# RKlompUU/fhe-regex

Hardware: AMD Instinct MI355X
Metric: TFHE gate-bootstraps/sec; end-to-end match time for /abc/ on 256-char content (higher is better)
Workload: dtype u64

## Files before the change

fhe-regex_amd/csrc/device.h:

```cpp
#pragma once
#include <cstdint>
#include <vector>

#include "common.h"
#include "owned.h"

namespace fr {

constexpr int MAX_OUT = 8;
enum : int32_t { JOB_MULTI = 0, JOB_DIRECT = 1, JOB_SIGN = 2 };
struct DevGate {
    int32_t n_in;
    int32_t offset;
    int32_t in_slot[16];
    int32_t in_w[16];
    int32_t n_out;
    int32_t direct;
    int32_t out_slot[MAX_OUT];
    uint8_t lut[MAX_OUT][16];
};
static_assert(sizeof(DevGate) == 304, "DevGate layout");
int lut_w_norm2(const uint8_t* lut);

struct DeviceTimers {
// ... 37 lines not shown
    void pack_bools(const DevGate* gates, size_t n, uint64_t* out_host);
    void pack_bools_compact(const DevGate* gates, size_t n, uint16_t* out_host );
    const double* pack_ms() const { return pack_ms_; }
    void encrypt_to_slots(const ClientKey& ck, const uint8_t* msgs, size_t count, const RngKey& key, uint64_t first_block,
                          const int* slots);

    Slots expand_to_slots(const RngKey& mask_key, uint64_t first_block, const uint8_t* bodies, size_t count);
    double expand_ms() const { return expand_ms_; }

    int alloc_slot();
    void free_slot(int s);
    void write_slots(const int* slots, size_t n, const uint64_t* host );
    void read_slot(int slot, uint64_t* host );
    void slots_to_device(const int* slots, size_t n, uint64_t* dst);
    void device_to_slots(const int* slots, size_t n, const uint64_t* src);
    void slots_to_device_async(const int* slots, size_t n, uint64_t* dst);
    void* stream() const { return cur().stream.get(); }
    void zero_slot(int slot);
    size_t arena_slots() const { return next_slot_; }
    size_t arena_free_slots() const { return free_slots_.size(); }

    void run_level(const DevGate* gates, size_t n);
    void run_level_resident(const DevGate* d_gates, const DevGate* host, size_t n, size_t n_refs = 0);
    gpu::DevBuf<DevGate> upload_gates(const DevGate* gates, size_t n, size_t n_refs = 0);
    void bind_content(const int* cmap, size_t n);
    void run_linear(const DevGate& g);
    void sync();

    void set_lanes(int n);
    int match_lanes() const { return (int)lanes_.size(); }
    void enter_lane(int i);
    void leave_lane();
    void set_profiling(int level) { profiling_ = level; }
    DeviceTimers& timers() { return timers_; }

    void keyswitch_host(const uint64_t* in, size_t count, uint64_t* out);
    void blind_rotate_host(const uint64_t* ks_in, const uint8_t* luts, size_t count, uint64_t* out);
    void blind_rotate_multi_host(const uint64_t* ks_in, const uint8_t* luts, int n_out, int direct, uint64_t* out);
    void ring_mul_host(const uint64_t* a, const uint64_t* b, size_t count, uint64_t* out);
    void bench_pbs(const std::vector<DevGate>& gates, int iters, double* br_ms, double* total_ms);

    std::string info() const;

  private:
    struct LaneState {
        gpu::Stream stream;
        gpu::DevBuf<uint64_t> ks;
        gpu::DevBuf<int8_t> dig;
        gpu::DevBuf<DevGate> pk_gates;
        gpu::DevBuf<int8_t> pk_dig;
        gpu::DevBuf<uint64_t> pk_g;
        gpu::DevBuf<uint16_t> pk_c16;
        gpu::DevBuf<double> kpre;
        gpu::StagingRing<int> cmap;
        size_t cmap_n = 0;
        gpu::Event done_ev;
        bool pending = false;
    };
    LaneState lane0_;
    std::vector<LaneState> lanes_;
    int lane_ = 0;
    LaneState& cur() { return lane_ ? lanes_[lane_ - 1] : lane0_; }
    const LaneState& cur() const { return lane_ ? lanes_[lane_ - 1] : lane0_; }
    bool lanes_pending_ = false;
    bool lanes_unsynced_ = false;
    gpu::Event main_ev_;
    std::vector<int> deferred_free_;
    hipStream_t cur_stream();
    void join_lanes();
    void sync_all();
    void ensure_arena(size_t slots);
    void ensure_ks(size_t n);
    void ensure_gates(size_t n);
    void validate_gates(const DevGate* gates, size_t n, size_t n_refs = 0) const;
    void launch_level(const DevGate* d_gates, const DevGate* host, size_t n);
    gpu::Event take_event();
    void resolve_timers();
    void ensure_digits(size_t rows);
    struct LimbKey {
        gpu::DevBuf<uint64_t> rows;
        gpu::DevBuf<int8_t> limbs;
        int KD = 0, ncols = 0, nlc = 0;
        explicit operator bool() const { return rows && limbs; }
        void alloc_rows(int kd, int nc) {
            limbs.reset();
            KD = kd, ncols = nc, nlc = ((nc * 8 + 127) / 128) * 128;
            rows.alloc((size_t)kd * nc);
        }
        void reset() { rows.reset(), limbs.reset(); }
    };
    void build_limbs(LimbKey& key);
    void drop_server_key() {
        ksk_.reset(), d_tbsk_.reset(), d_bsk_.reset(), d_fbsk_[0].reset(), d_fbsk_[1].reset();
        lane0_.kpre.reset();
        for (auto& l : lanes_) l.kpre.reset();
    }
    void drop_packing_key() { pksk_.reset(); }
    struct KsShape {
        int MR;
        size_t padded;
        int MC = 1, GZ = 1;
        bool lds = true;
    };
    KsShape ks_shape(size_t n) const {
        const int MR = n >= ks_mr4_min_ ? 4 : 1;
        return {MR, (n + 32 * MR - 1) / (32 * MR) * (32 * MR)};
    }
    template <int KSB, int KSL>
    void launch_ks_digits(const DevGate* d_gates, size_t n, size_t padded, int8_t* dig, uint64_t* out, int out_n,
                          int out_stride, hipEvent_t ev_start);
    void launch_limb_gemm(const int8_t* dig, const LimbKey& key, size_t n, const KsShape& sh, uint64_t* out,
                          int out_stride, hipEvent_t ev_stop);
    void launch_ks(const DevGate* d_gates, size_t n, uint64_t* d_ks, hipEvent_t ev_start = nullptr,
                   hipEvent_t ev_stop = nullptr);
    void launch_br(const DevGate* d_gates, const uint64_t* d_ks, size_t n, hipEvent_t ev_start = nullptr,
                   hipEvent_t ev_stop = nullptr);
    void run_br_jobs(const uint64_t* ks_in, std::vector<DevGate>& gates, uint64_t* out);
    void init_rns();
    void upload_rns_bsk(const std::vector<uint64_t>& bsk);
    void launch_br_rns(const DevGate* d_gates, const uint64_t* d_ks, size_t n, hipEvent_t ev_start, hipEvent_t ev_stop);
    void init_ks();
    void init_fft();
    void upload_fft_bsk(const std::vector<uint64_t>& bsk);
    void launch_br_fft(const DevGate* d_gates, const uint64_t* d_ks, size_t n, hipStream_t stream,
                       hipEvent_t ev_start = nullptr, hipEvent_t ev_stop = nullptr);
    void build_fourier_bsk();
    double key_load_ms_[5] = {0, 0, 0, 0, 0};
    double pk_load_ms_[3] = {0, 0, 0};
    gpu::StagingRing<uint8_t> xstage_;
    double expand_ms_ = 0;
    void stage_slot_list(const int* slots, size_t n);
    gpu::DevBuf<int> d_slot_list_;

    Params p_;
    int dev_;
    int e_ = 8;
    int e_small_ = 8;
    size_t small_batch_ = 256;
    LimbKey ksk_;
    gpu::DevBuf<uint64_t> d_tbsk_;
    LimbKey pksk_;
    double pack_ms_[4] = {0, 0, 0, 0};
    void pack_launch(const DevGate* gates, size_t n, uint64_t* out_words, uint16_t* out_c16);
    int pk_split_ = 0;
    bool ks_mfma_ = true;
    size_t ks_mr4_min_ = 96;
    int ks_mc_ = 0;
    int ks_split_ = 0;
    int ks_xcd_ = 1;
    bool ks_dig16_ = true;
    bool ks_lds_ = true;
    gpu::DevBuf<uint32_t> d_bsk_;
    gpu::DevBuf<uint32_t> d_tw_;
    int fft_e_ = 4;
    size_t fft_small_ = 256;
    size_t fft_pair_ = SIZE_MAX;
    bool fft_dual_ = false;
    size_t fft_kpre_ = 32;
    gpu::DevBuf<double> d_fbsk_[2];
    static int fbsk_index(int E) { return E == 4 ? 0 : 1; }
    bool fbsk_needed(int E) const { return E == 4 || E == fft_e_; }
    gpu::DevBuf<double> d_ftw_;
    gpu::DevBuf<double> d_fqt_;
    gpu::DevBuf<uint16_t> d_fleaf_;
    gpu::DevBuf<uint64_t> d_arena_;
    std::vector<int> free_slots_;
    size_t next_slot_ = 0;
    gpu::StagingRing<DevGate> gates_;
    struct PendingTimer {
        gpu::Event ev[4];
        size_t gates, outs;
        bool lat, pair, ks;
        bool chain;
    };
    bool latency_shape(size_t n) const;
    bool pair_shape(size_t n) const;
    std::vector<PendingTimer> pending_;
    std::vector<gpu::Event> event_pool_;
    int profiling_ = 0;
    bool timer_chain_ = true;
    DeviceTimers timers_;
    gpu::Event ev_[4];
};

}
```

fhe-regex_amd/csrc/fft_br.hip:

```cpp
#include <hip/hip_ext.h>
#include <hip/hip_runtime.h>

#include <cstring>

#include "device_impl.h"
#include "fft.h"
#include "geo.h"

namespace fr {

template <int M, int E>
using FGeo = NttGeo<M, E, 3, fft_layout_variant(ilog2c(M), ilog2c(E))>;
template <int M, int E>
constexpr int FV = fft_layout_variant(ilog2c(M), ilog2c(E));

__device__ __forceinline__ void cfwd(double2& x, double2& y, double2 c) { fft::fwd_bf(x.x, x.y, y.x, y.y, c.x, c.y); }
__device__ __forceinline__ void cinv(double2& u, double2& v, double2 c) { fft::inv_bf(u.x, u.y, v.x, v.y, c.x, c.y); }

template <int M, int E>
constexpr bool fradix4() {
    return E == 4 && FGeo<M, E>::LOG % 2 == 0;
}
template <int M, int E>
struct FTwr {
    static constexpr int COUNT = fradix4<M, E>() ? FGeo<M, E>::NPH * 3 : FGeo<M, E>::LOG * (E / 2);
    double2 v[COUNT];
};
__device__ __forceinline__ double2 fmul_i(double2 c) { return make_double2(-c.y, c.x); }
__device__ __forceinline__ void cinv_r4(double2 (&x)[4], double2 c, double2 ca, double2 cc) {
    fft::inv_r4(x[0].x, x[0].y, x[1].x, x[1].y, x[2].x, x[2].y, x[3].x, x[3].y, c.x, c.y, ca.x, ca.y, cc.x, cc.y);
}
template <class G, int E, int p, bool REV, class F>
__device__ __forceinline__ void for_butterflies(F&& fn) {
#pragma unroll
    for (int i = 0; i < G::s_end(p) - G::s_begin(p); ++i) {
        const int s = REV ? G::s_end(p) - 1 - i : G::s_begin(p) + i;
        const int dm = 1 << (G::LOG - 1 - s - G::lo(p));
#pragma unroll
        for (int m = 0; m < E; ++m) {
            if (m & dm) continue;
            fn(s, m, dm);
        }
    }
}
template <class G, int p>
__device__ __forceinline__ double2 ftw_at(const double2* tw, int b, int s, int m) {
    return (tw + (b >> (G::LOG - s)))[(1 << s) + (G::template moff<p>(m) >> (G::LOG - s))];
}
template <int M, int E, int p>
__device__ __forceinline__ void ftw_r4(const double2* tw, int tl, double2& c, double2& ca) {
    using G = FGeo<M, E>;
    constexpr int s0 = G::s_begin(p), s1 = s0 + 1;
    const int b = G::template base<p>(tl);
    c = ftw_at<G, p>(tw, b, s0, 0);
    ca = ftw_at<G, p>(tw, b, s1, 0);
// ... 399 lines not shown
        if (src < 0) {
            src += N;
            d = -d;
        }
        acc += (uint64_t)d * row[src];
    }
    return acc;
}

template <int M, int E>
__device__ __forceinline__ void fbr_publish(uint64_t* arow, const double (&alo)[E], const double (&ahi)[E], int tl) {
#pragma unroll
    for (int m = 0; m < E; ++m) {
        const int j = FGeo<M, E>::template idx<0>(tl, m);
        arow[j] = fft::torus_of_acc(alo[m]);
        arow[j + M] = fft::torus_of_acc(ahi[m]);
    }
}
template <int N>
__device__ __forceinline__ void fbr_terms(int tid, int n_out, int kind, const uint8_t* lut, uint32_t* wterms, int* wcnt) {
    if (tid < n_out && kind == JOB_MULTI) wcnt[tid] = lut_terms<N>(lut + 16 * tid, wterms + 16 * tid);
}
template <int N, int K, int NT>
__device__ __forceinline__ void fbr_outputs(int tid, const uint64_t* ab, const DevGate& gate, int n_out, int kind,
                                            const uint32_t* wterms, const int* wcnt, uint64_t* arena, int slot_stride) {
    constexpr int big = K * N;
    if (kind != JOB_MULTI) {
        uint64_t* out = arena + (size_t)gate.out_slot[0] * slot_stride;
        const uint64_t post = kind == JOB_SIGN ? (1ULL << (DELTA_LOG - 1)) : 0;
        for (int c = tid; c <= big; c += NT) {
            const ExtractIdx x = extract_index<N, K>(c);
            const uint64_t v = ab[x.pp * N + x.j];
            out[c] = (x.neg ? (uint64_t)0 - v : v) + (c == big ? post : 0);
        }
        return;
    }
    for (int f = 0; f < n_out; ++f) {
        const uint32_t* tf = wterms + 16 * f;
        const int nt = wcnt[f];
        uint64_t* out = arena + (size_t)gate.out_slot[f] * slot_stride;
        for (int c = tid; c <= big; c += NT) {
            const ExtractIdx x = extract_index<N, K>(c);
            const uint64_t v = w_step64<N>(ab + x.pp * N, tf, nt, x.j);
            out[c] = x.neg ? (uint64_t)0 - v : v;
        }
    }
}

template <int N, int K>
constexpr uint32_t kpre_step_bytes() {
    return 16u * (uint32_t)((K + 1) * (K + 1) * (N / 2));
}

template <int N, int K, int E, bool LAT, int B, bool KP>
__device__ __forceinline__ void fbr_rotate(const uint64_t* ks, int ks_stride, int n, const DevGate* gates, int n_gates,
                                           const double2* bsk, const double2* tw_g, const double2* psi_g,
                                           const uint16_t* leaf_g, uint64_t* arena, int slot_stride, const double2* kpre) {
    constexpr int M = N / 2;
    static_assert(!KP || (LAT && B == 1 && K == 1 && E == 4), "key products: the k = 1 latency shape");
    using G = FGeo<M, E>;
    static_assert(fexchanges_conflict_free<M, E>(), "LDS maps must make every exchange conflict-free");
    static_assert(G::base_matches_geo(), "base<p> must be the index map the LDS-map proofs reason about");
    static_assert(G::key_slot_matches_idx(), "the Fourier key's lane layout is the last-phase layout");
    static_assert(!LAT || E == 4, "the latency shape holds a step's GGSW values in registers: E = 4");
    static_assert(B == 1 || (B == 2 && LAT && K == 1 && E == 4), "pair shape: the k = 1 latency geometry");
    constexpr int NB = E >= 4 ? E / 4 : 1;
    constexpr int T = M / E, NT = (K + 1) * T, LAST = G::NPH - 1, XL = G::XL;
    constexpr int LOG2N2 = G::LOG + 2;
    constexpr bool TWR = fbr_twr<K, LAT>();
    constexpr int BS = (K + 1) * G::NP;
    constexpr bool PSIQ = !LAT || B > 1;
    extern __shared__ __attribute__((aligned(16))) double2 fsm[];
    double2* xbuf = fsm;
    double2* ibuf = LAT ? xbuf + B * BS : xbuf;
    double2* tw = xbuf + (LAT ? 2 : 1) * B * BS;
    constexpr int NPSI = KP ? 0 : PSIQ ? N / 2 : 2 * N;
    double2* psi = tw + (B == 1 ? M : 0);
    double2* twc = psi + NPSI;
    constexpr int NTWC = fbr_twc_entries<N, K, E, LAT>();
    uint8_t* lut = (uint8_t*)(twc + NTWC);
    uint16_t* abar = (uint16_t*)(lut + B * 16 * MAX_OUT);
    uint32_t* wterms = B == 1 ? (uint32_t*)(abar + 1026) : (uint32_t*)ibuf;
    int* wcnt = (int*)(wterms + B * 16 * MAX_OUT);
    uint16_t* nxt = B == 1 ? (uint16_t*)(wcnt + MAX_OUT) : abar + B * 1026;

    const int tid = threadIdx.x;
    const int P = __builtin_amdgcn_readfirstlane(tid / T), tl = tid % T;
    int gb[B];
    bool has[B];
    const uint64_t* in[B];
    int n_out[B], kind[B];
#pragma unroll
    for (int b = 0; b < B; ++b) {
        const int gi = B * (int)blockIdx.x + b;
        has[b] = gi < n_gates;
        gb[b] = has[b] ? gi : B * (int)blockIdx.x;
        in[b] = ks + (size_t)gb[b] * ks_stride;
        n_out[b] = gates[gb[b]].n_out;
        kind[b] = gates[gb[b]].direct;
    }
    if constexpr (B == 1)
        for (int i = tid; i < M; i += NT) tw[i] = tw_g[i];
    for (int i = tid; i < NPSI; i += NT) psi[psi_slot(i)] = psi_g[i];
    for (int i = 1 + tid; i < NTWC; i += NT) {
        const int s0 = 31 - __builtin_clz((unsigned)i), b = i - (1 << s0);
        if (s0 & 1) continue;
        const double2 c = tw_g[i], ca = tw_g[(2 << s0) + 2 * b];
        fft::cmul(c.x, c.y, ca.x, ca.y, twc[i].x, twc[i].y);
    }
    uint32_t bbar[B];
#pragma unroll
    for (int b = 0; b < B; ++b) {
        uint8_t* lb = lut + b * 16 * MAX_OUT;
        uint16_t* ab = abar + b * 1026;
        for (int i = tid; i < 16 * n_out[b]; i += NT) lb[i] = gates[gb[b]].lut[i / 16][i % 16];
        for (int i = tid; i < n; i += NT) ab[i] = (uint16_t)mod_switch(in[b][i], LOG2N2);
        if (tid == 0) ab[n] = 0;
        bbar[b] = mod_switch(in[b][n], LOG2N2);
    }
    uint32_t Lb[NB];
#pragma unroll
    for (int bb = 0; bb < NB; ++bb)
        Lb[bb] = (1u + 4u * (__brev((uint32_t)G::template idx<LAST>(tl, 4 * bb)) >> (32 - G::LOG))) & (uint32_t)(M - 1);
    __syncthreads();

    double alo[B][E], ahi[B][E];
#pragma unroll
    for (int b = 0; b < B; ++b) {
        const bool direct = kind[b] == JOB_DIRECT;
#pragma unroll
        for (int m = 0; m < E; ++m) {
            const int j = G::template idx<0>(tl, m);
            uint64_t v[2];
#pragma unroll
            for (int h = 0; h < 2; ++h) {
                const int s = (j + h * M + (int)bbar[b]) & (2 * N - 1);
                const uint64_t tv = test_poly<N>(s & (N - 1), direct, lut + b * 16 * MAX_OUT);
                v[h] = s < N ? tv : (uint64_t)0 - tv;
            }
            alo[b][m] = P == K ? fft::acc_of_torus(v[0]) : 0.0;
            ahi[b][m] = P == K ? fft::acc_of_torus(v[1]) : 0.0;
        }
    }

    double2* row = xbuf + P * G::NP;
    double2* irow = ibuf + P * G::NP;
    const int bl = G::template base<LAST>(tl);
    double2* row_bl = row + G::template at<XL>(bl);
    const double2* orow_bl[K];
#pragma unroll
    for (int q = 0; q < K; ++q) orow_bl[q] = xbuf + other_row<K>(P, q) * G::NP + G::template at<XL>(bl);
    constexpr uint32_t GG = (uint32_t)(K + 1) * (K + 1) * M;
    const __amdgpu_buffer_rsrc_t rs = bsk_rsrc(bsk);
    const uint32_t lane_off = 16u * (uint32_t)tl;
    const int steps = (n + 1) / 2;
    double2 gv[3][K + 1][LAT && !KP ? E : 1];
    double2 kv[K + 1][KP ? E : 1];
    FTwr<M, TWR ? E : 2> twr;
    if constexpr (TWR) ftw_load_phase<M, E, 0, B == 1 ? false : FR_TW_SGPR_PAIR>(twr, B == 1 ? tw : tw_g, tl);
#ifdef FR_BR_TIMING
    uint64_t tseg[6] = {0, 0, 0, 0, 0, 0};
    uint64_t tlast = __builtin_amdgcn_s_memtime();
    const uint64_t tstart = tlast;
#endif
    auto load_ggsw = [&](int gg, int tt) {
        if constexpr (!KP) {
            const uint32_t sb = (uint32_t)__builtin_amdgcn_readfirstlane(tt) * (3u * GG * 16u);
#pragma unroll
            for (int m = 0; m < E; ++m) {
                gv[gg][0][m] =
                    bsk_load(rs, lane_off, sb + 16u * (gg * GG + (uint32_t)(P * (K + 1) + P) * M + (uint32_t)m * T));
#pragma unroll
                for (int q = 0; q < K; ++q)
                    gv[gg][1 + q][m] = bsk_load(
                        rs, lane_off,
                        sb + 16u * (gg * GG + (uint32_t)(other_row<K>(P, q) * (K + 1) + P) * M + (uint32_t)m * T));
            }
        }
    };
    const __amdgpu_buffer_rsrc_t rk =
        bsk_rsrc(KP ? kpre + (size_t)blockIdx.x * ((size_t)((n + 1) / 2) * (kpre_step_bytes<N, K>() / 16)) : bsk);
    auto load_kp = [&](int tt) {
        if constexpr (KP) {
            const uint32_t sb = (uint32_t)__builtin_amdgcn_readfirstlane(tt) * kpre_step_bytes<N, K>();
#pragma unroll
            for (int r = 0; r <= K; ++r)
#pragma unroll
                for (int m = 0; m < E; ++m)
                    kv[r][m] = bsk_load(rk, lane_off, sb + 16u * (uint32_t)(((P * (K + 1) + r) * E + m) * T));
        }
    };
    constexpr int NPF = KP ? 0 : LAT ? (B > 1 ? FR_PAIR_PF : K == 1 ? FR_LAT_PF : FR_LAT_PF2) : 0;
    constexpr bool LATPF = NPF > 0;
    auto idle = [&](int t) {
        uint32_t z = 0;
#pragma unroll
        for (int b = 0; b < B; ++b) z |= abar[b * 1026 + 2 * t] | abar[b * 1026 + 2 * t + 1];
        return z == 0;
    };
    if constexpr (LATPF || KP) {
        for (int t = tid; t <= steps; t += NT) {
            int tt = t;
            while (tt < steps && idle(tt)) ++tt;
            nxt[t] = (uint16_t)tt;
        }
        __syncthreads();
        const int t0 = __builtin_amdgcn_readfirstlane((int)nxt[0]);
        for (int gg = 0; gg < NPF; ++gg) load_ggsw(gg, t0 < steps ? t0 : 0);
        load_kp(t0 < steps ? t0 : 0);
    }
    for (int t = 0; t < steps; ++t) {
        if (idle(t)) continue;
        BR_STAMP(0);
        const uint32_t sbase = (uint32_t)__builtin_amdgcn_readfirstlane(t) * (3u * GG * 16u);
        constexpr int G_TOP = !LAT || KP || B > 1 ? 3 : (NPF < 2 || K == 1) ? NPF : 3;
        constexpr int G_L1 = !LAT || KP ? 3 : B > 1 ? NPF : G_TOP + 1 < 3 ? G_TOP + 1 : 3;
        constexpr int G_L2 = !LAT || KP ? 3 : B > 1 ? (NPF + 1 < 3 ? NPF + 1 : 3) : G_TOP == 3 ? NPF : G_TOP + 2 < 3 ? G_TOP + 2 : 3;
        constexpr int PH_L1 = B > 1 ? FR_PAIR_LOAD : FR_LAT_LOAD1;
        constexpr int PH_L2 = B > 1 ? FR_PAIR_LOAD2 : FR_LAT_LOAD2;
        static_assert(G_L1 >= 3 || PH_L1 < G::NPH, "FR_PAIR_LOAD / FR_LAT_LOAD1 past the last forward phase");
        static_assert(G_L2 >= 3 || PH_L2 < G::NPH, "FR_PAIR_LOAD2 / FR_LAT_LOAD2 past the last forward phase");
        if constexpr (G_TOP < 3) {
            __builtin_amdgcn_sched_barrier(0);
            load_ggsw(G_TOP, t);
            __builtin_amdgcn_sched_barrier(0);
        }
        uint32_t ei[B], ej[B];
#pragma unroll
        for (int b = 0; b < B; ++b) {
            ei[b] = __builtin_amdgcn_readfirstlane((uint32_t)abar[b * 1026 + 2 * t]);
            ej[b] = __builtin_amdgcn_readfirstlane((uint32_t)abar[b * 1026 + 2 * t + 1]);
        }
        double bre[B][2][NB], bim[B][2][NB];
        auto psi_factors = [&]() {
#pragma unroll
            for (int b = 0; b < B; ++b)
#pragma unroll
                for (int h = 0; h < 2; ++h)
#pragma unroll
                    for (int bb = 0; bb < NB; ++bb)
                        key_psi_base<N, PSIQ>(psi, h == 0 ? ei[b] : ej[b], Lb[bb], bre[b][h][bb], bim[b][h][bb]);
        };
        if constexpr (LAT && B == 1 && !KP) psi_factors();
        double2 x[B][E];
#pragma unroll
        for (int b = 0; b < B; ++b)
#pragma unroll
            for (int m = 0; m < E; ++m)
                x[b][m] = make_double2(fft::acc_digit<23>(alo[b][m]), fft::acc_digit<23>(ahi[b][m]));
        BR_STAMP(1);
        fforward_from<M, E, 0, LAT, TWR, B, BS>(x, row, twr, tw, tl, [&](auto ph) {
            if constexpr (LAT) {
                constexpr int p = decltype(ph)::value;
                if constexpr (p == PH_L1 && G_L1 < 3) {
                    __builtin_amdgcn_sched_barrier(0);
                    load_ggsw(G_L1, t);
                    __builtin_amdgcn_sched_barrier(0);
                }
                if constexpr (p == PH_L2 && G_L2 < 3) {
                    __builtin_amdgcn_sched_barrier(0);
                    load_ggsw(G_L2, t);
                    __builtin_amdgcn_sched_barrier(0);
                }
            }
// ... 5 lines not shown
            for (int m = 0; m < E; ++m) row_bl[b * BS + G::template at<XL>(G::template moff<LAST>(m))] = x[b][m];
        constexpr bool AHEAD = !LAT && E == 8;
        constexpr bool PRE0 = !LAT;
        double2 Bc[3][K + 1];
        if constexpr (PRE0) load_slot<M, T, K>(Bc, rs, sbase, P, 0, lane_off);
        __syncthreads();
        if constexpr (!LAT || B > 1) psi_factors();
#pragma unroll
        for (int m = 0; m < E; ++m) {
            double2 Bn[3][K + 1];
            if constexpr (AHEAD) {
                if (m + 1 < E) load_slot<M, T, K>(Bn, rs, sbase, P, m + 1, lane_off);
                __builtin_amdgcn_sched_barrier(0);
            } else if constexpr (!LAT) {
                if (!PRE0 || m > 0) load_slot<M, T, K>(Bc, rs, sbase, P, m, lane_off);
            }
#pragma unroll
            for (int b = 0; b < B; ++b) {
                const double2 own = x[b][m];
                double2 oth[K];
#pragma unroll
                for (int q = 0; q < K; ++q) oth[q] = orow_bl[q][b * BS + G::template at<XL>(G::template moff<LAST>(m))];
                double kor, koi, kxr[K], kxi[K];
                if constexpr (KP) {
                    kor = kv[0][m].x, koi = kv[0][m].y;
#pragma unroll
                    for (int q = 0; q < K; ++q) kxr[q] = kv[1 + q][m].x, kxi[q] = kv[1 + q][m].y;
                } else {
                    const uint32_t sm = ((m & 1) << 1) | ((m >> 1) & 1);
                    auto key_at = [&](int gg, int r) __attribute__((always_inline)) {
                        return LAT ? gv[gg][r][LAT ? m : 0] : Bc[gg][r];
                    };
                    key_products<K>(bre[b], bim[b], m >> 2, ei[b], ej[b], sm, key_at, kor, koi, kxr, kxi);
                }
                double zr, zi;
                fft::cmul(own.x, own.y, kor, koi, zr, zi);
#pragma unroll
                for (int q = 0; q < K; ++q) fft::cmac(oth[q].x, oth[q].y, kxr[q], kxi[q], zr, zi);
                x[b][m] = make_double2(zr, zi);
            }
            if constexpr (!LAT) {
                __builtin_amdgcn_sched_barrier(0);
            }
            if constexpr (AHEAD) {
#pragma unroll
                for (int gg = 0; gg < 3; ++gg)
#pragma unroll
                    for (int r = 0; r <= K; ++r) Bc[gg][r] = Bn[gg][r];
            }
        }
        if constexpr (LATPF || KP) {
            const int tn = __builtin_amdgcn_readfirstlane((int)nxt[t + 1]);
            __builtin_amdgcn_sched_barrier(0);
            for (int gg = 0; gg < NPF; ++gg) load_ggsw(gg, tn < steps ? tn : t);
            load_kp(tn < steps ? tn : t);
            __builtin_amdgcn_sched_barrier(0);
        }
        BR_STAMP(3);
        finverse_from<M, E, LAST, LAT, TWR, B, BS>(x, irow, twr, tw, twc, tl);
        BR_STAMP(4);
#pragma unroll
        for (int b = 0; b < B; ++b)
#pragma unroll
            for (int m = 0; m < E; ++m) {
                alo[b][m] = fft::acc_reduce<23>(alo[b][m] + x[b][m].x);
                ahi[b][m] = fft::acc_reduce<23>(ahi[b][m] + x[b][m].y);
            }
        BR_STAMP(5);
    }
#ifdef FR_BR_TIMING
    if (blockIdx.x == 0 && tid == 0)
        printf("FBR_TIMING E=%d LAT=%d steps=%d total=%lu digits=%lu fwd=%lu mac=%lu inv=%lu acc=%lu top=%lu\n", E, (int)LAT,
               steps, (unsigned long)(__builtin_amdgcn_s_memtime() - tstart), (unsigned long)tseg[1],
               (unsigned long)tseg[2], (unsigned long)tseg[3], (unsigned long)tseg[4], (unsigned long)tseg[5],
               (unsigned long)tseg[0]);
#endif

    __syncthreads();
    uint64_t* accs = (uint64_t*)xbuf;
    static_assert(B == 1 || 8 * B * (K + 1) * N <= 16 * B * BS, "pair shape: u64 rows inside the forward rows");
#pragma unroll
    for (int b = 0; b < B; ++b) {
        fbr_publish<M, E>(accs + (b * (K + 1) + P) * N, alo[b], ahi[b], tl);
        fbr_terms<N>(tid, n_out[b], kind[b], lut + b * 16 * MAX_OUT, wterms + b * 16 * MAX_OUT, wcnt + b * MAX_OUT);
    }
    __syncthreads();
#pragma unroll
    for (int b = 0; b < B; ++b)
        if (has[b])
            fbr_outputs<N, K, NT>(tid, accs + b * (K + 1) * N, gates[gb[b]], n_out[b], kind[b], wterms + b * 16 * MAX_OUT,
                                  wcnt + b * MAX_OUT, arena, slot_stride);
}

template <int N, int K, int E, bool LAT, int B = 1>
__global__ void __launch_bounds__((fbr_threads<N, K, E>()), (fbr_min_waves<N, K, E, LAT>()))
k_blind_rotate_fft(const uint64_t* __restrict__ ks, int ks_stride, int n, const DevGate* __restrict__ gates,
                   int n_gates, const double2* __restrict__ bsk, const double2* __restrict__ tw_g,
                   const double2* __restrict__ psi_g, const uint16_t* __restrict__ leaf_g, uint64_t* __restrict__ arena,
                   int slot_stride) {
    fbr_rotate<N, K, E, LAT, B, false>(ks, ks_stride, n, gates, n_gates, bsk, tw_g, psi_g, leaf_g, arena, slot_stride,
                                       nullptr);
}
template <int N, int K, int E, bool LAT, int B = 1>
__global__ void __launch_bounds__((fbr_threads<N, K, E>()), (fbr_min_waves<N, K, E, LAT>()))
k_blind_rotate_fft_kp(const uint64_t* __restrict__ ks, int ks_stride, int n, const DevGate* __restrict__ gates,
                      int n_gates, const double2* __restrict__ tw_g, uint64_t* __restrict__ arena, int slot_stride,
                      const double2* __restrict__ kpre) {
    fbr_rotate<N, K, E, LAT, B, true>(ks, ks_stride, n, gates, n_gates, nullptr, tw_g, nullptr, nullptr, arena,
                                      slot_stride, kpre);
}

template <int N>
__global__ void __launch_bounds__(N / 8)
k_key_products(const uint64_t* __restrict__ ks, int ks_stride, int n, int n_gates, const double2* __restrict__ bsk,
               const double2* __restrict__ psi_g, double2* __restrict__ kpre) {
    constexpr int K = 1, E = 4, M = N / 2, T = M / E;
    using G = FGeo<M, E>;
    static_assert(G::key_slot_matches_idx(), "the Fourier key's lane layout is the last-phase layout");
    constexpr int LAST = G::NPH - 1, LOG2N2 = G::LOG + 2;
    constexpr uint32_t GG = (uint32_t)(K + 1) * (K + 1) * M;
    __shared__ __attribute__((aligned(16))) double2 psi[N / 2];
    const int tl = threadIdx.x, t = (int)blockIdx.x, P = (int)blockIdx.y;
    const int steps = (n + 1) / 2;
    for (int i = tl; i < N / 2; i += T) psi[psi_slot(i)] = psi_g[i];
    const __amdgpu_buffer_rsrc_t rs = bsk_rsrc(bsk);
    const uint32_t lane_off = 16u * (uint32_t)tl, sb = (uint32_t)t * (3u * GG * 16u);
    double2 gv[3][K + 1][E];
#pragma unroll
    for (int gg = 0; gg < 3; ++gg)
#pragma unroll
        for (int m = 0; m < E; ++m) {
            gv[gg][0][m] = bsk_load(rs, lane_off, sb + 16u * (gg * GG + (uint32_t)(P * (K + 1) + P) * M + (uint32_t)m * T));
            gv[gg][1][m] = bsk_load(
                rs, lane_off, sb + 16u * (gg * GG + (uint32_t)(other_row<K>(P, 0) * (K + 1) + P) * M + (uint32_t)m * T));
        }
    const uint32_t Lb = (1u + 4u * (__brev((uint32_t)G::template idx<LAST>(tl, 0)) >> (32 - G::LOG))) & (uint32_t)(M - 1);
    __syncthreads();
    for (int b = 0; b < n_gates; ++b) {
        const uint64_t* in = ks + (size_t)b * ks_stride;
        const uint32_t ei = (uint16_t)mod_switch(in[2 * t], LOG2N2);
        const uint32_t ej = 2 * t + 1 < n ? (uint16_t)mod_switch(in[2 * t + 1], LOG2N2) : 0u;
        if ((ei | ej) == 0) continue;
        double br[2][1], bi[2][1];
        key_psi_base<N, true>(psi, ei, Lb, br[0][0], bi[0][0]);
        key_psi_base<N, true>(psi, ej, Lb, br[1][0], bi[1][0]);
        double2* out = kpre + (((size_t)b * steps + t) * (K + 1) + P) * ((K + 1) * M) + tl;
#pragma unroll
        for (int m = 0; m < E; ++m) {
            const uint32_t sm = ((m & 1) << 1) | ((m >> 1) & 1);
            double kor, koi, kxr[K], kxi[K];
            key_products<K>(br, bi, 0, ei, ej, sm, [&](int gg, int r) __attribute__((always_inline)) { return gv[gg][r][m]; },
                            kor, koi, kxr, kxi);
            out[m * T] = make_double2(kor, koi);
            out[(E + m) * T] = make_double2(kxr[0], kxi[0]);
        }
    }
}

#ifndef FR_BR_PAIR_TU
extern template __global__ void k_blind_rotate_fft<2048, 1, 4, true, 2>(const uint64_t*, int, int, const DevGate*, int,
                                                                         const double2*, const double2*, const double2*,
                                                                         const uint16_t*, uint64_t*, int);
#endif

template <int N>
constexpr size_t fbr_dual_smem_bytes() {
    return 16 * (2 * (size_t)FGeo<N / 2, 4>::NP + (size_t)N / 2) + 16 * MAX_OUT + 2 * 1026 + 4 * 16 * MAX_OUT +
           4 * MAX_OUT;
}
template <int N>
__global__ void __launch_bounds__(N / 8, 2)
k_blind_rotate_fft_dual(const uint64_t* __restrict__ ks, int ks_stride, int n, const DevGate* __restrict__ gates,
                        int n_gates, const double2* __restrict__ bsk, const double2* __restrict__ tw_g,
                        const double2* __restrict__ psi_g, const uint16_t* __restrict__ leaf_g,
                        uint64_t* __restrict__ arena, int slot_stride) {
    constexpr int K = 1, E = 4, M = N / 2, B = 2;
    using G = FGeo<M, E>;
    static_assert(fexchanges_conflict_free<M, E>(), "LDS maps must make every exchange conflict-free");
    static_assert(G::base_matches_geo(), "base<p> must be the index map the LDS-map proofs reason about");
    static_assert(G::key_slot_matches_idx(), "the Fourier key's lane layout is the last-phase layout");
    static_assert(fradix4<M, E>(), "dual shape: the k = 1 geometry (radix-4 inverse)");
    constexpr int T = M / E, NT = T, LAST = G::NPH - 1;
    constexpr int LOG2N2 = G::LOG + 2;
    constexpr int BS = G::NP;
    extern __shared__ __attribute__((aligned(16))) double2 fsm[];
    double2* xbuf = fsm;
    double2* psi = xbuf + B * BS;
    uint8_t* lut = (uint8_t*)(psi + N / 2);
    uint16_t* abar = (uint16_t*)(lut + 16 * MAX_OUT);
    uint32_t* wterms = (uint32_t*)(abar + 1026);
    int* wcnt = (int*)(wterms + 16 * MAX_OUT);

    const int tl = threadIdx.x;
    const int gi = (int)blockIdx.x;
    const uint64_t* in = ks + (size_t)gi * ks_stride;
    const int n_out = gates[gi].n_out, kind = gates[gi].direct;
    for (int i = tl; i < N / 2; i += NT) psi[psi_slot(i)] = psi_g[i];
    for (int i = tl; i < 16 * n_out; i += NT) lut[i] = gates[gi].lut[i / 16][i % 16];
    for (int i = tl; i < n; i += NT) abar[i] = (uint16_t)mod_switch(in[i], LOG2N2);
    if (tl == 0) abar[n] = 0;
    const uint32_t bbar = mod_switch(in[n], LOG2N2);
    const uint32_t Lb = (1u + 4u * (__brev((uint32_t)G::template idx<LAST>(tl, 0)) >> (32 - G::LOG))) & (uint32_t)(M - 1);
    __syncthreads();

    double alo[B][E], ahi[B][E];
    {
        const bool direct = kind == JOB_DIRECT;
#pragma unroll
        for (int m = 0; m < E; ++m) {
// ... 90 lines not shown
                    for (int r = 0; r < 2; ++r)
#pragma unroll
                        for (int c = 0; c < 2; ++c) Bc[gg][r][c] = Bn[gg][r][c];
            }
        }
        finverse_from<M, E, LAST, false, true, B, BS>(x, xbuf, twr, nullptr, nullptr, tl);
#pragma unroll
        for (int P = 0; P < B; ++P)
#pragma unroll
            for (int m = 0; m < E; ++m) {
                alo[P][m] = fft::acc_reduce<23>(alo[P][m] + x[P][m].x);
                ahi[P][m] = fft::acc_reduce<23>(ahi[P][m] + x[P][m].y);
            }
    }

    __syncthreads();
    uint64_t* accs = (uint64_t*)xbuf;
    static_assert(8 * B * N <= 16 * B * BS, "dual shape: u64 rows inside the exchange rows");
#pragma unroll
    for (int P = 0; P < B; ++P) fbr_publish<M, E>(accs + P * N, alo[P], ahi[P], tl);
    fbr_terms<N>(tl, n_out, kind, lut, wterms, wcnt);
    __syncthreads();
    if (gi >= n_gates) return;
    fbr_outputs<N, K, NT>(tl, accs, gates[gi], n_out, kind, wterms, wcnt, arena, slot_stride);
}

#ifndef FR_BR_PAIR_TU
constexpr bool fft_supported(int K, int N, int E) {
    return (K == 1 && N == 2048 && E == 4) || (K == 2 && N == 1024 && (E == 4 || E == 8));
}

template <int N, int K, int E, bool LAT, int B = 1>
static void fft_attr() {
    static_assert(fbr_smem_bytes<N, K, E, LAT, B>() <= (LAT ? 160 * 1024 : 160 * 1024 / fbr_tp_groups<K, E>()),
                  "LDS per workgroup of the shape");
    HIP_CHECK(hipFuncSetAttribute((const void*)k_blind_rotate_fft<N, K, E, LAT, B>,
                                  hipFuncAttributeMaxDynamicSharedMemorySize, (int)fbr_smem_bytes<N, K, E, LAT, B>()));
}

template <class F>
static void fft_dispatch(const Params& p, F&& body) {
    if (p.k == 1 && p.N == 2048) body(std::integral_constant<int, 2048>{}, std::integral_constant<int, 1>{});
    else if (p.k == 2 && p.N == 1024) body(std::integral_constant<int, 1024>{}, std::integral_constant<int, 2>{});
    else throw Error(FR_ERR_INVALID, "device: FFT ring needs (k, N) in {(1, 2048), (2, 1024)}");
}

void Device::init_fft() {
    if (p_.k == 2) fft_e_ = 8;
    if (const char* ev = std::getenv("FR_FFT_LANE_ELEMS")) fft_e_ = std::atoi(ev);
    if (const char* ev = std::getenv("FR_FFT_SMALL_BATCH")) fft_small_ = (size_t)std::atol(ev);
    if (const char* ev = std::getenv("FR_FFT_PAIR_BATCH")) fft_pair_ = (size_t)std::atol(ev);
    if (const char* ev = std::getenv("FR_FFT_DUAL")) fft_dual_ = std::atoi(ev) != 0;
    if (const char* ev = std::getenv("FR_FFT_KPRE_BATCH")) fft_kpre_ = (size_t)std::atol(ev);
    if (p_.k != 1) fft_pair_ = 0, fft_kpre_ = 0;
    if (!fft_supported(p_.k, p_.N, fft_e_))
        throw Error(FR_ERR_INVALID, "device: FFT ring needs (k, N, E) in {(1, 2048, 4), (2, 1024, 4 or 8)}");
    fft_dispatch(p_, [&](auto nc, auto kc) {
        constexpr int N = decltype(nc)::value, K = decltype(kc)::value;
        fft_attr<N, K, 4, true>();
        fft_attr<N, K, 4, false>();
        if constexpr (K == 1) {
            fft_attr<N, K, 4, true, 2>();
            static_assert(fbr_smem_bytes<N, K, 4, true, 1, true>() <= 160 * 1024, "LDS per workgroup of the shape");
            HIP_CHECK(hipFuncSetAttribute((const void*)k_blind_rotate_fft_kp<N, K, 4, true, 1>,
                                          hipFuncAttributeMaxDynamicSharedMemorySize,
                                          (int)fbr_smem_bytes<N, K, 4, true, 1, true>()));
            static_assert(fbr_dual_smem_bytes<N>() <= 80 * 1024, "dual shape: two workgroups per CU");
            HIP_CHECK(hipFuncSetAttribute((const void*)k_blind_rotate_fft_dual<N>,
                                          hipFuncAttributeMaxDynamicSharedMemorySize, (int)fbr_dual_smem_bytes<N>()));
        }
        if constexpr (fft_supported(K, N, 8)) fft_attr<N, K, 8, false>();
    });

    fft::Tables T(p_.N);
    d_ftw_.alloc(2 * (size_t)T.M);
    std::vector<fft::c64> psi(2 * (size_t)p_.N);
    for (int k = 0; k < 2 * p_.N; ++k) psi[k] = fft::psi_pow(p_.N, k);
    d_fqt_.alloc(2 * psi.size());
    d_fleaf_.alloc((size_t)T.M);
    HIP_CHECK(hipMemcpy(d_ftw_.get(), T.tw.data(), 16 * (size_t)T.M, hipMemcpyHostToDevice));
    HIP_CHECK(hipMemcpy(d_fqt_.get(), psi.data(), 16 * psi.size(), hipMemcpyHostToDevice));
    HIP_CHECK(hipMemcpy(d_fleaf_.get(), T.leaf.data(), 2 * (size_t)T.M, hipMemcpyHostToDevice));
}

void Device::upload_fft_bsk(const std::vector<uint64_t>& bsk) {
    const int N = p_.N, M = N / 2, kp1 = p_.k + 1;
    const size_t polys = p_.bsk_ggsw() * (size_t)kp1 * kp1;
    fft::Tables tabs(N);
    std::vector<fft::c64> four;
    fft::bsk_to_fourier(tabs, bsk, polys, four);
    std::vector<fft::c64> lanes(four.size());
    for (int E : {8, 4}) {
        gpu::DevBuf<double>& dst = d_fbsk_[fbsk_index(E)];
        dst.reset();
        if (!fft_supported(p_.k, N, E) || !fbsk_needed(E)) continue;
        const int T = M / E, e = ilog2c(E);
        std::vector<int> slot((size_t)M);
        for (int q = 0; q < M; ++q) slot[q] = fft_key_slot(tabs.LOG, e, q % T, q / T);
        for (size_t pq = 0; pq < polys; ++pq)
            for (size_t q = 0; q < (size_t)M; ++q) lanes[pq * M + q] = four[pq * M + slot[q]];
        dst.alloc(2 * lanes.size());
        HIP_CHECK(hipMemcpy(dst.get(), lanes.data(), 16 * lanes.size(), hipMemcpyHostToDevice));
    }
}

void Device::launch_br_fft(const DevGate* d_gates, const uint64_t* d_ks, size_t n, hipStream_t s, hipEvent_t ev_start,
                           hipEvent_t ev_stop) {
    auto launch = [&](auto kernel, size_t grid, int threads, size_t lds, int E) {
        hipExtLaunchKernelGGL(kernel, dim3((unsigned)grid), dim3(threads), (uint32_t)lds, s, ev_start, ev_stop, 0, d_ks,
                              p_.ks_stride(), p_.n, d_gates, (int)n, (const double2*)d_fbsk_[fbsk_index(E)].get(),
                              (const double2*)d_ftw_.get(), (const double2*)d_fqt_.get(),
                              (const uint16_t*)d_fleaf_.get(), d_arena_.get(), p_.slot_stride());
    };
    fft_dispatch(p_, [&](auto nc, auto kc) {
        constexpr int N = decltype(nc)::value, K = decltype(kc)::value;
        auto go = [&](auto ec, auto lat, auto bc) {
            constexpr int E = decltype(ec)::value;
            constexpr bool LAT = decltype(lat)::value;
            constexpr int B = decltype(bc)::value;
            if constexpr (fft_supported(K, N, E) && (B == 1 || K == 1))
                launch(k_blind_rotate_fft<N, K, E, LAT, B>, (n + B - 1) / B, fbr_threads<N, K, E>(),
                       fbr_smem_bytes<N, K, E, LAT, B>(), E);
        };
        using I4 = std::integral_constant<int, 4>;
        using I8 = std::integral_constant<int, 8>;
        using B1 = std::integral_constant<int, 1>;
        if (n <= fft_small_ && n <= fft_kpre_ && K == 1) {
            if constexpr (K == 1) {
                const int steps = (p_.n + 1) / 2;
                const size_t per = (size_t)steps * (kpre_step_bytes<N, K>() / 8);
                gpu::DevBuf<double>& kpre = cur().kpre;
                if (kpre.size() < n * per) {
                    HIP_CHECK(hipStreamSynchronize(s));
                    kpre.alloc(n * per);
                }
                hipExtLaunchKernelGGL(k_key_products<N>, dim3((unsigned)steps, K + 1), dim3(N / 8), 0, s, ev_start,
                                      nullptr, 0, d_ks, p_.ks_stride(), p_.n, (int)n,
                                      (const double2*)d_fbsk_[fbsk_index(4)].get(), (const double2*)d_fqt_.get(),
                                      (double2*)kpre.get());
                hipExtLaunchKernelGGL((k_blind_rotate_fft_kp<N, K, 4, true, 1>), dim3((unsigned)n),
                                      dim3(fbr_threads<N, K, 4>()), (uint32_t)fbr_smem_bytes<N, K, 4, true, 1, true>(), s,
                                      nullptr, ev_stop, 0, d_ks, p_.ks_stride(), p_.n, d_gates, (int)n,
                                      (const double2*)d_ftw_.get(), d_arena_.get(), p_.slot_stride(),
                                      (const double2*)kpre.get());
            }
        } else if (n <= fft_small_) go(I4{}, std::true_type{}, B1{});
        else if (n <= fft_pair_ && K == 1 && fft_dual_) {
            if constexpr (K == 1) launch(k_blind_rotate_fft_dual<N>, n, N / 8, fbr_dual_smem_bytes<N>(), 4);
        } else if (n <= fft_pair_) go(I4{}, std::true_type{}, std::integral_constant<int, 2>{});
        else if (fft_e_ == 4) go(I4{}, std::false_type{}, B1{});
        else go(I8{}, std::false_type{}, B1{});
    });
    HIP_CHECK(hipGetLastError());
}

#endif

}
```

Measured before the change: 124,700.

## Overlap key-product precompute with blind rotation by splitting steps into two launches

The small-batch key-products path now computes key products for the first S steps up front, in a kernel split over gate chunks. A combined kernel then runs blind rotation over steps [0,S) while extra workgroups produce key products for the remaining steps. A second launch finishes rotation over [S,steps), carrying accumulators through a new global carry buffer. The key-product kernel also loads mod-switched pairs once per 64 gates and broadcasts them with readlane. The aim is to hide the serial precompute latency behind rotation, at the cost of an extra launch, carry traffic, and a heuristic split point built from hardcoded microsecond constants.

After: 125,600 (median of 6 runs). No clear change (+0.7%).

```diff
diff --git a/fhe-regex_amd/csrc/device.h b/fhe-regex_amd/csrc/device.h
--- a/fhe-regex_amd/csrc/device.h
+++ b/fhe-regex_amd/csrc/device.h
@@ -113,6 +113,7 @@
         gpu::DevBuf<uint64_t> pk_g;
         gpu::DevBuf<uint16_t> pk_c16;
         gpu::DevBuf<double> kpre;
+        gpu::DevBuf<double> kcarry;
         gpu::StagingRing<int> cmap;
         size_t cmap_n = 0;
         gpu::Event done_ev;
@@ -218,6 +219,8 @@
     size_t fft_pair_ = SIZE_MAX;
     bool fft_dual_ = false;
     size_t fft_kpre_ = 32;
+    int fft_kpre_split_ = -1;
+    int kpre_split(size_t n, int steps) const;
     gpu::DevBuf<double> d_fbsk_[2];
     static int fbsk_index(int E) { return E == 4 ? 0 : 1; }
     bool fbsk_needed(int E) const { return E == 4 || E == fft_e_; }
diff --git a/fhe-regex_amd/csrc/fft_br.hip b/fhe-regex_amd/csrc/fft_br.hip
--- a/fhe-regex_amd/csrc/fft_br.hip
+++ b/fhe-regex_amd/csrc/fft_br.hip
@@ -1,6 +1,7 @@
 #include <hip/hip_ext.h>
 #include <hip/hip_runtime.h>
 
+#include <cmath>
 #include <cstring>
 
 #include "device_impl.h"
@@ -506,12 +507,14 @@
     return 16u * (uint32_t)((K + 1) * (K + 1) * (N / 2));
 }
 
-template <int N, int K, int E, bool LAT, int B, bool KP>
+template <int N, int K, int E, bool LAT, int B, bool KP, bool PART = false>
 __device__ __forceinline__ void fbr_rotate(const uint64_t* ks, int ks_stride, int n, const DevGate* gates, int n_gates,
                                            const double2* bsk, const double2* tw_g, const double2* psi_g,
-                                           const uint16_t* leaf_g, uint64_t* arena, int slot_stride, const double2* kpre) {
+                                           const uint16_t* leaf_g, uint64_t* arena, int slot_stride, const double2* kpre,
+                                           int t_begin = 0, int t_end = 0, double2* carry = nullptr) {
     constexpr int M = N / 2;
     static_assert(!KP || (LAT && B == 1 && K == 1 && E == 4), "key products: the k = 1 latency shape");
+    static_assert(!PART || KP, "step ranges: the key-products variant");
     using G = FGeo<M, E>;
     static_assert(fexchanges_conflict_free<M, E>(), "LDS maps must make every exchange conflict-free");
     static_assert(G::base_matches_geo(), "base<p> must be the index map the LDS-map proofs reason about");
@@ -579,21 +582,32 @@
     __syncthreads();
 
     double alo[B][E], ahi[B][E];
-#pragma unroll
-    for (int b = 0; b < B; ++b) {
-        const bool direct = kind[b] == JOB_DIRECT;
-#pragma unroll
-        for (int m = 0; m < E; ++m) {
-            const int j = G::template idx<0>(tl, m);
-            uint64_t v[2];
-#pragma unroll
-            for (int h = 0; h < 2; ++h) {
-                const int s = (j + h * M + (int)bbar[b]) & (2 * N - 1);
-                const uint64_t tv = test_poly<N>(s & (N - 1), direct, lut + b * 16 * MAX_OUT);
-                v[h] = s < N ? tv : (uint64_t)0 - tv;
-            }
-            alo[b][m] = P == K ? fft::acc_of_torus(v[0]) : 0.0;
-            ahi[b][m] = P == K ? fft::acc_of_torus(v[1]) : 0.0;
+    double2* cw = nullptr;
+    if constexpr (PART) cw = carry + (size_t)blockIdx.x * (E * NT) + tid;
+    if (!PART || t_begin == 0) {
+#pragma unroll
+        for (int b = 0; b < B; ++b) {
+            const bool direct = kind[b] == JOB_DIRECT;
+#pragma unroll
+            for (int m = 0; m < E; ++m) {
+                const int j = G::template idx<0>(tl, m);
+                uint64_t v[2];
+#pragma unroll
+                for (int h = 0; h < 2; ++h) {
+                    const int s = (j + h * M + (int)bbar[b]) & (2 * N - 1);
+                    const uint64_t tv = test_poly<N>(s & (N - 1), direct, lut + b * 16 * MAX_OUT);
+                    v[h] = s < N ? tv : (uint64_t)0 - tv;
+                }
+                alo[b][m] = P == K ? fft::acc_of_torus(v[0]) : 0.0;
+                ahi[b][m] = P == K ? fft::acc_of_torus(v[1]) : 0.0;
+            }
+        }
+    } else if constexpr (PART) {
+#pragma unroll
+        for (int q = 0; q < E / 2; ++q) {
+            const double2 lo = cw[q * NT], hi = cw[(E / 2 + q) * NT];
+            alo[0][2 * q] = lo.x, alo[0][2 * q + 1] = lo.y;
+            ahi[0][2 * q] = hi.x, ahi[0][2 * q + 1] = hi.y;
         }
     }
 
@@ -608,6 +622,7 @@
     const __amdgpu_buffer_rsrc_t rs = bsk_rsrc(bsk);
     const uint32_t lane_off = 16u * (uint32_t)tl;
     const int steps = (n + 1) / 2;
+    const int tb = PART ? t_begin : 0, te = PART ? t_end : steps;
     double2 gv[3][K + 1][LAT && !KP ? E : 1];
     double2 kv[K + 1][KP ? E : 1];
     FTwr<M, TWR ? E : 2> twr;
@@ -659,11 +674,11 @@
             nxt[t] = (uint16_t)tt;
         }
         __syncthreads();
-        const int t0 = __builtin_amdgcn_readfirstlane((int)nxt[0]);
-        for (int gg = 0; gg < NPF; ++gg) load_ggsw(gg, t0 < steps ? t0 : 0);
-        load_kp(t0 < steps ? t0 : 0);
-    }
-    for (int t = 0; t < steps; ++t) {
+        const int t0 = __builtin_amdgcn_readfirstlane((int)nxt[tb]);
+        for (int gg = 0; gg < NPF; ++gg) load_ggsw(gg, t0 < te ? t0 : tb);
+        load_kp(t0 < te ? t0 : tb);
+    }
+    for (int t = tb; t < te; ++t) {
         if (idle(t)) continue;
         BR_STAMP(0);
         const uint32_t sbase = (uint32_t)__builtin_amdgcn_readfirstlane(t) * (3u * GG * 16u);
@@ -775,8 +790,8 @@
         if constexpr (LATPF || KP) {
             const int tn = __builtin_amdgcn_readfirstlane((int)nxt[t + 1]);
             __builtin_amdgcn_sched_barrier(0);
-            for (int gg = 0; gg < NPF; ++gg) load_ggsw(gg, tn < steps ? tn : t);
-            load_kp(tn < steps ? tn : t);
+            for (int gg = 0; gg < NPF; ++gg) load_ggsw(gg, tn < te ? tn : t);
+            load_kp(tn < te ? tn : t);
             __builtin_amdgcn_sched_barrier(0);
         }
         BR_STAMP(3);
@@ -799,6 +814,16 @@
                (unsigned long)tseg[0]);
 #endif
 
+    if constexpr (PART) {
+        if (t_end < steps) {
+#pragma unroll
+            for (int q = 0; q < E / 2; ++q) {
+                cw[q * NT] = make_double2(alo[0][2 * q], alo[0][2 * q + 1]);
+                cw[(E / 2 + q) * NT] = make_double2(ahi[0][2 * q], ahi[0][2 * q + 1]);
+            }
+            return;
+        }
+    }
     __syncthreads();
     uint64_t* accs = (uint64_t*)xbuf;
     static_assert(B == 1 || 8 * B * (K + 1) * N <= 16 * B * BS, "pair shape: u64 rows inside the forward rows");
@@ -834,18 +859,16 @@
 }
 
 template <int N>
-__global__ void __launch_bounds__(N / 8)
-k_key_products(const uint64_t* __restrict__ ks, int ks_stride, int n, int n_gates, const double2* __restrict__ bsk,
-               const double2* __restrict__ psi_g, double2* __restrict__ kpre) {
+__device__ __forceinline__ void key_products_step(double2* psi, int fid, int fn, int t, int P, int tl, const uint64_t* ks,
+                                                  int ks_stride, int n, int b_lo, int b_hi, const double2* bsk,
+                                                  const double2* psi_g, double2* kpre) {
     constexpr int K = 1, E = 4, M = N / 2, T = M / E;
     using G = FGeo<M, E>;
     static_assert(G::key_slot_matches_idx(), "the Fourier key's lane layout is the last-phase layout");
     constexpr int LAST = G::NPH - 1, LOG2N2 = G::LOG + 2;
     constexpr uint32_t GG = (uint32_t)(K + 1) * (K + 1) * M;
-    __shared__ __attribute__((aligned(16))) double2 psi[N / 2];
-    const int tl = threadIdx.x, t = (int)blockIdx.x, P = (int)blockIdx.y;
     const int steps = (n + 1) / 2;
-    for (int i = tl; i < N / 2; i += T) psi[psi_slot(i)] = psi_g[i];
+    for (int i = fid; i < N / 2; i += fn) psi[psi_slot(i)] = psi_g[i];
     const __amdgpu_buffer_rsrc_t rs = bsk_rsrc(bsk);
     const uint32_t lane_off = 16u * (uint32_t)tl, sb = (uint32_t)t * (3u * GG * 16u);
     double2 gv[3][K + 1][E];
@@ -859,25 +882,62 @@
         }
     const uint32_t Lb = (1u + 4u * (__brev((uint32_t)G::template idx<LAST>(tl, 0)) >> (32 - G::LOG))) & (uint32_t)(M - 1);
     __syncthreads();
-    for (int b = 0; b < n_gates; ++b) {
-        const uint64_t* in = ks + (size_t)b * ks_stride;
-        const uint32_t ei = (uint16_t)mod_switch(in[2 * t], LOG2N2);
-        const uint32_t ej = 2 * t + 1 < n ? (uint16_t)mod_switch(in[2 * t + 1], LOG2N2) : 0u;
-        if ((ei | ej) == 0) continue;
-        double br[2][1], bi[2][1];
-        key_psi_base<N, true>(psi, ei, Lb, br[0][0], bi[0][0]);
-        key_psi_base<N, true>(psi, ej, Lb, br[1][0], bi[1][0]);
-        double2* out = kpre + (((size_t)b * steps + t) * (K + 1) + P) * ((K + 1) * M) + tl;
-#pragma unroll
-        for (int m = 0; m < E; ++m) {
-            const uint32_t sm = ((m & 1) << 1) | ((m >> 1) & 1);
-            double kor, koi, kxr[K], kxi[K];
-            key_products<K>(br, bi, 0, ei, ej, sm, [&](int gg, int r) __attribute__((always_inline)) { return gv[gg][r][m]; },
-                            kor, koi, kxr, kxi);
-            out[m * T] = make_double2(kor, koi);
-            out[(E + m) * T] = make_double2(kxr[0], kxi[0]);
-        }
-    }
+    for (int b0 = b_lo; b0 < b_hi; b0 += 64) {
+        uint32_t pairs = 0;
+        if (const int bm = b0 + (tl & 63); bm < b_hi) {
+            const uint64_t* in = ks + (size_t)bm * ks_stride;
+            const uint32_t ei = (uint16_t)mod_switch(in[2 * t], LOG2N2);
+            const uint32_t ej = 2 * t + 1 < n ? (uint16_t)mod_switch(in[2 * t + 1], LOG2N2) : 0u;
+            pairs = ei | (ej << 16);
+        }
+        const int b1 = b_hi - b0 < 64 ? b_hi : b0 + 64;
+        for (int b = b0; b < b1; ++b) {
+            const uint32_t pr = __builtin_amdgcn_readlane(pairs, b - b0);
+            const uint32_t ei = pr & 0xffffu, ej = pr >> 16;
+            if (pr == 0) continue;
+            double br[2][1], bi[2][1];
+            key_psi_base<N, true>(psi, ei, Lb, br[0][0], bi[0][0]);
+            key_psi_base<N, true>(psi, ej, Lb, br[1][0], bi[1][0]);
+            double2* out = kpre + (((size_t)b * steps + t) * (K + 1) + P) * ((K + 1) * M) + tl;
+    #pragma unroll
+            for (int m = 0; m < E; ++m) {
+                const uint32_t sm = ((m & 1) << 1) | ((m >> 1) & 1);
+                double kor, koi, kxr[K], kxi[K];
+                key_products<K>(br, bi, 0, ei, ej, sm, [&](int gg, int r) __attribute__((always_inline)) { return gv[gg][r][m]; },
+                                kor, koi, kxr, kxi);
+                out[m * T] = make_double2(kor, koi);
+                out[(E + m) * T] = make_double2(kxr[0], kxi[0]);
+            }
+        }
+    }
+}
+template <int N>
+__global__ void __launch_bounds__(N / 8)
+k_key_products(const uint64_t* __restrict__ ks, int ks_stride, int n, int n_gates, int b_chunk,
+               const double2* __restrict__ bsk, const double2* __restrict__ psi_g, double2* __restrict__ kpre) {
+    __shared__ __attribute__((aligned(16))) double2 psi[N / 2];
+    const int b_lo = (int)blockIdx.z * b_chunk, b_hi = b_lo + b_chunk < n_gates ? b_lo + b_chunk : n_gates;
+    key_products_step<N>(psi, (int)threadIdx.x, N / 8, (int)blockIdx.x, (int)blockIdx.y, (int)threadIdx.x, ks, ks_stride, n,
+                         b_lo, b_hi, bsk, psi_g, kpre);
+}
+template <int N, int K, int E, bool LAT, int B = 1, bool PRODUCE = true>
+__global__ void __launch_bounds__((fbr_threads<N, K, E>()), (fbr_min_waves<N, K, E, LAT>()))
+k_blind_rotate_fft_kp_part(const uint64_t* __restrict__ ks, int ks_stride, int n, const DevGate* __restrict__ gates,
+                           int n_gates, const double2* __restrict__ bsk, const double2* __restrict__ tw_g,
+                           const double2* __restrict__ psi_g, uint64_t* __restrict__ arena, int slot_stride, double2* kpre,
+                           double2* carry, int t_begin, int t_end) {
+    static_assert(fbr_smem_bytes<N, K, E, LAT, B, true>() >= 16 * (size_t)(N / 2), "the producer's psi table fits");
+    if (PRODUCE && (int)blockIdx.x >= n_gates) {
+        extern __shared__ __attribute__((aligned(16))) double2 fsm[];
+        constexpr int T = N / 2 / E;
+        const int tid = (int)threadIdx.x;
+        key_products_step<N>(fsm, tid, (K + 1) * T, t_end + ((int)blockIdx.x - n_gates),
+                             __builtin_amdgcn_readfirstlane(tid / T), tid % T, ks, ks_stride, n, 0, n_gates, bsk, psi_g,
+                             kpre);
+        return;
+    }
+    fbr_rotate<N, K, E, LAT, B, true, true>(ks, ks_stride, n, gates, n_gates, nullptr, tw_g, nullptr, nullptr, arena,
+                                            slot_stride, kpre, t_begin, t_end, carry);
 }
 
 #ifndef FR_BR_PAIR_TU
@@ -1074,6 +1134,7 @@
     if (const char* ev = std::getenv("FR_FFT_PAIR_BATCH")) fft_pair_ = (size_t)std::atol(ev);
     if (const char* ev = std::getenv("FR_FFT_DUAL")) fft_dual_ = std::atoi(ev) != 0;
     if (const char* ev = std::getenv("FR_FFT_KPRE_BATCH")) fft_kpre_ = (size_t)std::atol(ev);
+    if (const char* ev = std::getenv("FR_FFT_KPRE_SPLIT")) fft_kpre_split_ = std::atoi(ev);
     if (p_.k != 1) fft_pair_ = 0, fft_kpre_ = 0;
     if (!fft_supported(p_.k, p_.N, fft_e_))
         throw Error(FR_ERR_INVALID, "device: FFT ring needs (k, N, E) in {(1, 2048, 4), (2, 1024, 4 or 8)}");
@@ -1085,6 +1146,12 @@
             fft_attr<N, K, 4, true, 2>();
             static_assert(fbr_smem_bytes<N, K, 4, true, 1, true>() <= 160 * 1024, "LDS per workgroup of the shape");
             HIP_CHECK(hipFuncSetAttribute((const void*)k_blind_rotate_fft_kp<N, K, 4, true, 1>,
+                                          hipFuncAttributeMaxDynamicSharedMemorySize,
+                                          (int)fbr_smem_bytes<N, K, 4, true, 1, true>()));
+            HIP_CHECK(hipFuncSetAttribute((const void*)k_blind_rotate_fft_kp_part<N, K, 4, true, 1, true>,
+                                          hipFuncAttributeMaxDynamicSharedMemorySize,
+                                          (int)fbr_smem_bytes<N, K, 4, true, 1, true>()));
+            HIP_CHECK(hipFuncSetAttribute((const void*)k_blind_rotate_fft_kp_part<N, K, 4, true, 1, false>,
                                           hipFuncAttributeMaxDynamicSharedMemorySize,
                                           (int)fbr_smem_bytes<N, K, 4, true, 1, true>()));
             static_assert(fbr_dual_smem_bytes<N>() <= 80 * 1024, "dual shape: two workgroups per CU");
@@ -1124,6 +1191,14 @@
         dst.alloc(2 * lanes.size());
         HIP_CHECK(hipMemcpy(dst.get(), lanes.data(), 16 * lanes.size(), hipMemcpyHostToDevice));
     }
+}
+
+int Device::kpre_split(size_t n, int steps) const {
+    if (fft_kpre_split_ >= 0) return fft_kpre_split_ < steps ? fft_kpre_split_ : 0;
+    constexpr double KPRE_STEP_US = 2.7, KPRE_PROD_US0 = 13.0, KPRE_PROD_US1 = 3.9;
+    const double prod = KPRE_PROD_US0 + KPRE_PROD_US1 * (double)n;
+    const int S = (int)std::ceil(prod / (KPRE_STEP_US + prod / steps));
+    return S >= 1 && S < steps ? S : 0;
 }
 
 void Device::launch_br_fft(const DevGate* d_gates, const uint64_t* d_ks, size_t n, hipStream_t s, hipEvent_t ev_start,
@@ -1151,20 +1226,41 @@
             if constexpr (K == 1) {
                 const int steps = (p_.n + 1) / 2;
                 const size_t per = (size_t)steps * (kpre_step_bytes<N, K>() / 8);
+                constexpr size_t per_carry = 2 * (size_t)N;
                 gpu::DevBuf<double>& kpre = cur().kpre;
-                if (kpre.size() < n * per) {
+                gpu::DevBuf<double>& kcarry = cur().kcarry;
+                if (kpre.size() < n * per || kcarry.size() < n * per_carry) {
                     HIP_CHECK(hipStreamSynchronize(s));
                     kpre.alloc(n * per);
+                    kcarry.alloc(n * per_carry);
                 }
-                hipExtLaunchKernelGGL(k_key_products<N>, dim3((unsigned)steps, K + 1), dim3(N / 8), 0, s, ev_start,
-                                      nullptr, 0, d_ks, p_.ks_stride(), p_.n, (int)n,
-                                      (const double2*)d_fbsk_[fbsk_index(4)].get(), (const double2*)d_fqt_.get(),
-                                      (double2*)kpre.get());
-                hipExtLaunchKernelGGL((k_blind_rotate_fft_kp<N, K, 4, true, 1>), dim3((unsigned)n),
-                                      dim3(fbr_threads<N, K, 4>()), (uint32_t)fbr_smem_bytes<N, K, 4, true, 1, true>(), s,
-                                      nullptr, ev_stop, 0, d_ks, p_.ks_stride(), p_.n, d_gates, (int)n,
-                                      (const double2*)d_ftw_.get(), d_arena_.get(), p_.slot_stride(),
-                                      (const double2*)kpre.get());
+                const double2* d_bsk = (const double2*)d_fbsk_[fbsk_index(4)].get();
+                const int S = kpre_split(n, steps);
+                constexpr int KPRE_HEAD_CHUNK = 4;
+                const int chunk = S ? KPRE_HEAD_CHUNK : (int)n;
+                hipExtLaunchKernelGGL(k_key_products<N>,
+                                      dim3((unsigned)(S ? S : steps), K + 1, (unsigned)(((int)n + chunk - 1) / chunk)),
+                                      dim3(N / 8), 0, s, ev_start, nullptr, 0, d_ks, p_.ks_stride(), p_.n, (int)n, chunk,
+                                      d_bsk, (const double2*)d_fqt_.get(), (double2*)kpre.get());
+                if (S == 0) {
+                    hipExtLaunchKernelGGL((k_blind_rotate_fft_kp<N, K, 4, true, 1>), dim3((unsigned)n),
+                                          dim3(fbr_threads<N, K, 4>()), (uint32_t)fbr_smem_bytes<N, K, 4, true, 1, true>(),
+                                          s, nullptr, ev_stop, 0, d_ks, p_.ks_stride(), p_.n, d_gates, (int)n,
+                                          (const double2*)d_ftw_.get(), d_arena_.get(), p_.slot_stride(),
+                                          (const double2*)kpre.get());
+                } else {
+                    auto part = [&](auto produce, size_t grid, int t_begin, int t_end, hipEvent_t stop) {
+                        constexpr bool PRODUCE = decltype(produce)::value;
+                        hipExtLaunchKernelGGL((k_blind_rotate_fft_kp_part<N, K, 4, true, 1, PRODUCE>), dim3((unsigned)grid),
+                                              dim3(fbr_threads<N, K, 4>()),
+                                              (uint32_t)fbr_smem_bytes<N, K, 4, true, 1, true>(), s, nullptr, stop, 0, d_ks,
+                                              p_.ks_stride(), p_.n, d_gates, (int)n, d_bsk, (const double2*)d_ftw_.get(),
+                                              (const double2*)d_fqt_.get(), d_arena_.get(), p_.slot_stride(),
+                                              (double2*)kpre.get(), (double2*)kcarry.get(), t_begin, t_end);
+                    };
+                    part(std::true_type{}, n + (size_t)(steps - S), 0, S, nullptr);
+                    part(std::false_type{}, n, S, steps, ev_stop);
+                }
             }
         } else if (n <= fft_small_) go(I4{}, std::true_type{}, B1{});
         else if (n <= fft_pair_ && K == 1 && fft_dual_) {
```
